# HudsonAlpha/rust-msbwt

Measured on AMD Instinct MI355X. Metric: k-mer count queries/sec (whole node), higher is better.
Workload: dtype u64

## Files before the change

rust-msbwt_amd/csrc/lanes_kernel.hpp:

```cpp
#pragma once
#include <hip/hip_runtime.h>

#include <algorithm>
#include <cstdio>
#include <cstdlib>
#include <type_traits>

#include "kernels.hpp"
#include "rank_ops.hpp"
#include "search_common.hpp"
#include "sparse_table.hpp"

namespace msbwt {
namespace {

typedef __attribute__((address_space(3))) void lds_void;
typedef __attribute__((address_space(1))) const void global_void;

constexpr int kRing = 64;
#ifdef MSBWT_LANES_REGIONS
template <int kWords> constexpr int kRegionsFor = MSBWT_LANES_REGIONS;
#else
template <int kWords> constexpr int kRegionsFor = 10;
#endif
// ... 22 lines not shown

template <int kWords, bool kPlaced, bool kTier = false>
struct LaneScratchT {
    static constexpr int kMaxK = kWords * 32 / 3;
    static constexpr int kRegions = kRegionsFor<kWords>;
    static constexpr int kLineSlots = kRegions * 8;
    static constexpr uint32_t kMaxSecond = uint32_t(kLineSlots) - 64u;
    static_assert(kRegions >= 10 && kRegions % 2 == 0, "first-bound lines take 8 regions; regions come in padded pairs");
    uint4 lines[(kRegions / 2) * 136];
    RingItemT<kWords, kPlaced, kTier> ring[kRing];
    uint32_t cnt[kSearchCounters];
};
static_assert(sizeof(LaneScratchT<6, true>) <= 160 * 1024 / 12 && sizeof(LaneScratchT<6, false, true>) <= 160 * 1024 / 12 && sizeof(LaneScratchT<3, true, true>) <= 160 * 1024 / 12,
              "12 one-wave workgroups per CU (but for packed queries of k > 32 on a two-tier table: 8)");

__host__ __device__ constexpr uint32_t region_base(uint32_t i) { return 136u * (i >> 1) + 72u * (i & 1u); }

__device__ __forceinline__ uint32_t line_base(uint32_t s) { return region_base(s >> 3) + 8u * (s & 7u); }

__device__ __forceinline__ uint32_t xor_and(uint32_t a, uint32_t b, uint32_t c) { return __builtin_amdgcn_bitop3_b32(a, b, c, 0x28); }

struct PlaneLine {
    uint32_t m[8];
    uint32_t meta[8];
};

__device__ __forceinline__ void read_plane_line(const uint4 *lines, uint32_t slot, uint32_t s, PlaneLine &L) {
    const uint32_t base = line_base(slot), g = slot & 7u;
    const uint32_t x0 = (s & 1u) ? 0u : ~0u, x1 = (s & 2u) ? 0u : ~0u, x2 = (s & 4u) ? 0u : ~0u;
#pragma unroll
    for (uint32_t j = 0; j < 8; ++j) {
        const uint4 c = lines[base + (j ^ g)];
        L.m[j] = xor_and(c.z, x2, xor_and(c.y, x1, c.x ^ x0));
        L.meta[j] = c.w;
    }
}

__device__ __forceinline__ uint64_t plane_line_bound(const PlaneLine &L, uint32_t s, uint64_t pos) {
    const uint32_t r = uint32_t(pos) & 255u, idx = r >> 6;
    const uint64_t t = (1ull << (r & 63u)) - 1ull;
    uint32_t cnt = 0, lo = 0;
#pragma unroll
    for (uint32_t j = 0; j < 4; ++j) {
        const uint64_t mask = j < idx ? ~0ull : (j == idx ? t : 0ull);
        cnt += uint32_t(__popc(L.m[2 * j] & uint32_t(mask))) + uint32_t(__popc(L.m[2 * j + 1] & uint32_t(mask >> 32)));
    }
#pragma unroll
    for (uint32_t j = 0; j < 6; ++j) lo = (s == j) ? L.meta[j] : lo;
    const uint32_t hi = (((s >> 2) ? L.meta[7] : L.meta[6]) >> ((s & 3u) * 8u)) & 0xFFu;
    return ((uint64_t(hi) << 32) | lo) + cnt;
}

struct RunCont {
    uint32_t dword, at, acc;
};

__device__ __forceinline__ void run_dword(uint32_t x, uint32_t sx, uint32_t &all, uint32_t &mine) {
    const uint32_t lens = (x >> 3) & 0x1F1F1F1Fu, t = (x & 0x07070707u) ^ sx;
    const uint32_t other = ((t + 0x7F7F7F7Fu) | t) & 0x80808080u;
    const uint32_t match = ((other ^ 0x80808080u) >> 7) * 0xFFu;
    all = __builtin_amdgcn_sad_u8(lens, 0u, 0u);
    mine = __builtin_amdgcn_sad_u8(lens & match, 0u, 0u);
}

__device__ __forceinline__ uint32_t run_dword_clip(uint32_t x, uint32_t s, uint32_t at, uint32_t r) {
    uint32_t cnt = 0;
#pragma unroll
    for (int b = 0; b < 4; ++b) {
        const uint32_t run = (x >> (8 * b)) & 0xFFu, len = run >> 3;
        cnt += (run & 7u) == s ? uint32_t(min(max(int(r) - int(at), 0), int(len))) : 0u;
        at += len;
    }
    return cnt;
}

__device__ __forceinline__ void run_line_first(const uint4 *lines, uint32_t slot, uint32_t s, uint64_t pos, uint64_t &out, uint32_t &need, RunCont &cont) {
    const uint32_t base = line_base(slot), g = slot & 7u;
    const uint4 c0 = lines[base + (0u ^ g)], c1 = lines[base + (1u ^ g)];
    cont = RunCont{24u, 0u, 0u};
    if ((c1.w & 0x80000000u) != 0u) {
        need = lines[base + (2u ^ g)].x * 2u + 1u + ((uint32_t(pos) & 511u) >> 8);
        return;
    }
    const uint32_t lo = s == 0u ? c0.x : s == 1u ? c0.y : s == 2u ? c0.z : s == 3u ? c0.w : s == 4u ? c1.x : c1.y;
    const uint32_t hi = (((s >> 2) ? c1.w : c1.z) >> ((s & 3u) * 8u)) & 0xFFu;
    const uint32_t r0 = uint32_t(pos) & 511u, sx = s * 0x01010101u;
    uint32_t cnt = 0, cur = 0, str = 0;
#pragma unroll
    for (uint32_t j = 2; j < 8; ++j) {
        const uint4 c = lines[base + (j ^ g)];
        const uint32_t word[4] = {c.x, c.y, c.z, c.w};
#pragma unroll
        for (uint32_t i = 0; i < 4; ++i) {
            uint32_t all, mine;
            run_dword(word[i], sx, all, mine);
            const uint32_t end = cur + all;
            cnt += end <= r0 ? mine : 0u;
            const bool here = end > r0 && cont.dword == 24u;
            str = here ? word[i] : str;
            cont.at = here ? cur : cont.at;
            cont.dword = here ? 4u * (j - 2u) + i : cont.dword;
            cur = end;
        }
    }
    cont.acc = cnt;
    out = ((uint64_t(hi) << 32) | lo) + cnt + run_dword_clip(str, s, cont.at, r0);
}

__device__ __forceinline__ void run_line_continue(const uint4 *lines, uint32_t slot, uint32_t s, uint64_t pos, bool same_line, const RunCont &cont, uint64_t &out,
                                                  uint32_t &need) {
    const uint32_t base = line_base(slot), g = slot & 7u;
    const uint4 c0 = lines[base + (0u ^ g)], c1 = lines[base + (1u ^ g)];
    if ((c1.w & 0x80000000u) != 0u) {
        need = lines[base + (2u ^ g)].x * 2u + 1u + ((uint32_t(pos) & 511u) >> 8);
        return;
    }
    const uint32_t lo = s == 0u ? c0.x : s == 1u ? c0.y : s == 2u ? c0.z : s == 3u ? c0.w : s == 4u ? c1.x : c1.y;
    const uint32_t hi = (((s >> 2) ? c1.w : c1.z) >> ((s & 3u) * 8u)) & 0xFFu;
    const uint32_t r1 = uint32_t(pos) & 511u, sx = s * 0x01010101u;
    uint32_t d = same_line ? cont.dword : 0u, cur = same_line ? cont.at : 0u, acc = same_line ? cont.acc : 0u;
    const uint32_t *words = reinterpret_cast<const uint32_t *>(lines);
    while (d < 24u) {
        const uint32_t x = words[(base + ((2u + (d >> 2)) ^ g)) * 4u + (d & 3u)];
        uint32_t all, mine;
        run_dword(x, sx, all, mine);
        if (cur + all <= r1) {
            acc += mine;
            cur += all;
            ++d;
        } else {
            acc += run_dword_clip(x, s, cur, r1);
            break;
        }
    }
    out = ((uint64_t(hi) << 32) | lo) + acc;
}

struct PairLine {
    uint32_t m[4];
    uint32_t field;
};

__device__ __forceinline__ void read_pair_line(const uint4 *lines, uint32_t slot, uint32_t a2, uint32_t b2, PairLine &L) {
    const uint32_t base = line_base(slot), g = slot & 7u, p = a2 * 4u + b2;
    const uint4 a0 = lines[base + (0u ^ g)], a1 = lines[base + (1u ^ g)], b0 = lines[base + (2u ^ g)], b1 = lines[base + (3u ^ g)];
    const uint4 v = lines[base + (uint32_t(kPairValidChunk) ^ g)];
    const uint32_t na0 = (a2 & 1u) - 1u, na1 = ((a2 >> 1) & 1u) - 1u, nb0 = (b2 & 1u) - 1u, nb1 = ((b2 >> 1) & 1u) - 1u;
    L.m[0] = xor_and(b1.x, nb1, xor_and(b0.x, nb0, xor_and(a1.x, na1, xor_and(a0.x, na0, v.x))));
    L.m[1] = xor_and(b1.y, nb1, xor_and(b0.y, nb0, xor_and(a1.y, na1, xor_and(a0.y, na0, v.y))));
    L.m[2] = xor_and(b1.z, nb1, xor_and(b0.z, nb0, xor_and(a1.z, na1, xor_and(a0.z, na0, v.z))));
    L.m[3] = xor_and(b1.w, nb1, xor_and(b0.w, nb0, xor_and(a1.w, na1, xor_and(a0.w, na0, v.w))));
    const uint16_t *halves = reinterpret_cast<const uint16_t *>(lines + base + ((uint32_t(kPairLoChunk) + (p >> 3)) ^ g));
    const uint8_t *bytes = reinterpret_cast<const uint8_t *>(lines + base + (uint32_t(kPairHiChunk) ^ g));
    L.field = uint32_t(halves[p & 7u]) | (uint32_t(bytes[p]) << 16);
}

__device__ __forceinline__ uint32_t pair_line_count(const PairLine &L, uint32_t r) {
    const uint64_t t = (1ull << (r & 63u)) - 1ull;
    const bool upper = r >= 64u;
    const uint64_t lo = upper ? ~0ull : t, hi = upper ? t : 0ull;
    return uint32_t(__popc(L.m[0] & uint32_t(lo))) + uint32_t(__popc(L.m[1] & uint32_t(lo >> 32))) +
           uint32_t(__popc(L.m[2] & uint32_t(hi))) + uint32_t(__popc(L.m[3] & uint32_t(hi >> 32)));
}

__device__ __forceinline__ uint64_t pair_line_bound(const PairLine &L, uint64_t super_base, uint32_t r) {
    return super_base + L.field + pair_line_count(L, r);
}

enum SparseKernel : int { kDirectTable = 0, kSparseComplete = 1, kSparseTier = 2, kSparseWide = 3, kSparseXwide = 4 };

template <int kSparse>
__device__ __forceinline__ constexpr SparseLayout kernel_layout(uint32_t depth) {
    if constexpr (kSparse == kSparseTier) return sparse_layout(depth, true);
    else return kSparse == kSparseXwide ? kLayoutXwide : kSparse == kSparseWide ? kLayoutWide : kLayoutComplete;
}
static_assert(kLayoutTierWide.slots <= kLayoutTier.slots, "kernel_layout<kSparseTier>(kSparseMinDepth) has the most slots of its two");

template <uint32_t kMaxSlots>
__device__ __forceinline__ bool sparse_scan(const uint4 *lines, uint32_t slot, const SparseLayout &L, uint64_t want, uint64_t &l, uint32_t &width, uint32_t &header,
                                            bool &maybe) {
    const uint32_t base = line_base(slot), g = slot & 7u;
    const uint32_t *words = reinterpret_cast<const uint32_t *>(lines);
    const uint8_t *bytes = reinterpret_cast<const uint8_t *>(lines);
    auto word_at = [&](uint32_t w) -> uint32_t { return words[(base + ((w >> 2) ^ g)) * 4u + (w & 3u)]; };
    auto byte_at = [&](uint32_t b) -> uint32_t { return bytes[(base + ((b >> 4) ^ g)) * 16u + (b & 15u)]; };
    auto width_at = [&](uint32_t i) -> uint32_t { return L.width_byte ? byte_at(L.width_byte + i) : word_at(i) >> kSparseWidthShift; };
    auto take = [&](uint32_t i) {
        const uint32_t lo = word_at(L.l_lo_word + i), hi = byte_at(L.l_hi_byte + i);
// ... 130 lines not shown
    auto count_here = [&](int which, uint64_t ballot) {
        if (lane == uint32_t(__builtin_ctzll(__ballot(true)))) ws.cnt[which] += uint32_t(__popcll(ballot));
    };
    const uint32_t dma_group = lane >> 3, dma_chunk_bytes = ((lane & 7u) ^ dma_group) * 16u;

    const uint32_t ncounters = min(uint32_t(kTicketCounters), max(1u, gridDim.x >> 3));
    const uint32_t my_counter = (blockIdx.x >> 3) % ncounters;
    uint64_t static_next = (uint64_t(blockIdx.x) + gridDim.x) * grain;
    auto take_ticket = [&]() -> uint64_t {
        if (tile_counter == nullptr) {
            const uint64_t t = static_next;
            static_next += uint64_t(gridDim.x) * grain;
            return t;
        }
        unsigned long long t = 0;
        if (lane == 0) t = atomicAdd(tile_counter + my_counter * 16u, 1ull);
        const uint64_t drawn = (uint64_t(uint32_t(__builtin_amdgcn_readfirstlane(int(uint32_t(t >> 32))))) << 32) |
                               uint32_t(__builtin_amdgcn_readfirstlane(int(uint32_t(t))));
        return (uint64_t(gridDim.x) + my_counter + drawn * uint64_t(ncounters)) * grain;
    };
    uint64_t next_tile = uint64_t(blockIdx.x) * grain;
    uint32_t seg_left = grain;
    uint64_t seg_after = take_ticket();
    auto advance_tile = [&]() {
        ++next_tile;
        if (--seg_left == 0u) {
            next_tile = seg_after;
            seg_left = grain;
            seg_after = take_ticket();
        }
    };
    uint32_t ring_head = 0, ring_count = 0;
    uint64_t ring_tile = 0;
    uint32_t filter_pause = 0;

    bool have = false;
    bool tmode = false;
    uint32_t tdist = 0;
    bool tmaybe = false;
    bool dmode = false;
    uint32_t ovf_l = 0, ovf_h = 0;
    uint64_t l = 0, h = 0;
    uint32_t w[kWords], rem = 0;
    uint64_t qid = 0;
#pragma unroll
    for (int i = 0; i < kWords; ++i) w[i] = 0;

    uint4 staged_next[kPieces];
#pragma unroll
    for (int i = 0; i < kPieces; ++i) staged_next[i] = make_uint4(0, 0, 0, 0);
    const uint32_t wshift = (kReads && src.strands == 3u) ? 1u : 0u;
    const uint32_t tile_windows = uint32_t(kTile) >> wshift;
    const bool reads_fast = kReads && src.win_off == nullptr && src.windows >= tile_windows;
    const double inv_windows = kReads ? 1.0 / double(src.windows) : 0.0;
    uint32_t staged_n0 = 0;
    uint32_t staged_out = 0, prep_out = 0;
    const bool placed = kPacked && (src.out_index != nullptr || src.place_inline != 0u);
    auto place_of = [&](uint64_t v, uint32_t out) -> uint64_t { return placed ? uint64_t(out) : v; };
    auto fetch_tile_bytes = [&](uint64_t tile, auto first) {
        if (!kPacked && tile >= ntiles) return;
        if (!kReads) {
            if (decltype(first)::value && !kPacked && src.inline_n != 0u) {
                staged_next[0] = lane == 0u ? src.inline_kmer[0] : lane == 1u ? src.inline_kmer[1] : lane == 2u ? src.inline_kmer[2] : lane == 3u ? src.inline_kmer[3] : make_uint4(0, 0, 0, 0);
                return;
            }
            const uint64_t q0 = tile * kTile;
            if constexpr (kPacked) {
                constexpr uint32_t kOwn = kWords == 3 ? 1u : 2u;
                const uint32_t stride = src.packed_stride ? src.packed_stride : kOwn;
                const uint64_t qi = min(q0 + lane, n - 1u);
                const uint64_t *words = reinterpret_cast<const uint64_t *>(kmers) + qi * stride;
                const uint2 a = *reinterpret_cast<const uint2 *>(words);
                staged_next[0].x = a.x;
                staged_next[0].y = a.y;
                if constexpr (kWords == 6) {
                    const uint2 b = *reinterpret_cast<const uint2 *>(words + 1);
                    staged_next[0].z = b.x;
                    staged_next[0].w = b.y;
                }
                const uint32_t *place = src.place_inline != 0u ? reinterpret_cast<const uint32_t *>(words + kOwn)
                                        : src.out_index != nullptr ? src.out_index + qi : reinterpret_cast<const uint32_t *>(words);
                staged_out = *place;
                return;
            }
            const uint32_t nbytes = uint32_t(min(uint64_t(kTile), n - q0)) * k;
#pragma unroll
            for (int i = 0; i < kPieces; ++i) staged_next[i] = load_piece(kmers + q0 * k, nbytes, lane + 64u * i);
        } else if (reads_fast) {
            const uint64_t g0 = (tile * kTile) >> wshift;
            uint64_t r0 = uint64_t(double(g0) * inv_windows);
            int64_t w0 = int64_t(g0 - r0 * src.windows);
            if (w0 < 0) { --r0; w0 += src.windows; }
            if (w0 >= int64_t(src.windows)) { ++r0; w0 -= src.windows; }
            staged_n0 = min(tile_windows, src.windows - uint32_t(w0));
            const uint64_t at = r0 * src.read_len + uint64_t(w0) + 4u * lane, data_len = src.n_reads * src.read_len;
            uint32_t d = 0;
            if (at + 4u <= data_len) {
                __builtin_memcpy(&d, kmers + at, 4);
            } else {
                for (uint32_t b = 0; b < 4u; ++b)
                    if (at + b < data_len) d |= uint32_t(kmers[at + b]) << (8u * b);
            }
            staged_next[0].x = d;
        }
    };
    fetch_tile_bytes(next_tile, std::true_type{});
// ... 111 lines not shown
                        tmode = !dmode;
                    }
                }
                qid = ring_tile * kTile + (it.meta >> 24);
                if constexpr (kPacked) qid = place_of(qid, it.extra[RingItem::kOutAt]);
                ovf_l = ovf_h = 0u;
                have = true;
            }
            const uint32_t taken = min(ring_count, uint32_t(__popcll(idle)));
            ring_head = (ring_head + taken) & (kRing - 1);
            ring_count -= taken;
        }
        const bool broken = have && !(kSparse && tmode) && !(kTier && dmode) && (h > total || l > h);
        if (broken) {
            atomicOr(flags, kFlagInternal);
            if (debug != nullptr && atomicCAS(reinterpret_cast<unsigned long long *>(debug), 0ull, 1ull) == 0ull) {
                debug[1] = l;
                debug[2] = h;
                debug[3] = (uint64_t(rem) << 56) | qid;
                debug[4] = (uint64_t(w[1]) << 32) | w[0];
                debug[5] = (uint64_t(blockIdx.x) << 32) | lane;
            }
            if constexpr (kRange) store_range_raw(src, qid, ~0ull, ~0ull);
            else store_count<kReads>(src, qid, ~0ull);
            have = false;
        }
        busy = __ballot(have);

        if (!prepared && next_tile < ntiles) {
            if (counting && lane == 0u) ws.cnt[kCntWavesWorked] = 1u;
            const uint64_t tile = next_tile;
            advance_tile();
            const uint64_t q0 = tile * kTile;
            const uint32_t in_tile = uint32_t(min(uint64_t(kTile), n - q0));
            const bool filter_now = filter != nullptr && filter_pause == 0;
            bool looked_up = false, passed = false, filtered = false;
            const uint32_t tile_n0 = staged_n0;
            const uint4 packed_words = staged_next[0];
            if constexpr (kPacked) asm volatile("v_mov_b32 %0, %1" : "=v"(prep_out) : "v"(staged_out));
            if (kPacked) {
            } else if (!kReads) {
#pragma unroll
                for (int i = 0; i < kPieces; ++i) ws.lines[kStageLead / 16 + lane + 64u * i] = staged_next[i];
            } else if (reads_fast) {
                const uint32_t d = staged_next[0].x;
                uint32_t f = 0, c = 0;
#pragma unroll
                for (uint32_t b = 0; b < 4u; ++b) {
                    uint32_t sym = (d >> (8u * b)) & 0xFFu;
                    if (src.ascii) sym = ascii_to_code(sym);
                    f |= sym << (8u * b);
                    c |= complement_code(sym) << (8u * (3u - b));
                }
                uint32_t *codes = reinterpret_cast<uint32_t *>(ws.lines) + kStageLead / 4;
                codes[lane] = f;
                codes[64u + (63u - lane)] = c;
            }
            wave_lds_sync();
            prep_kind = 0;
            prep_tile = tile;
            if (lane < in_tile) {
                PackedQuery<kWords> pq;
                if (kPacked) {
                    pack_two_bit<kWords>(k, depth, (uint64_t(packed_words.y) << 32) | packed_words.x, (uint64_t(packed_words.w) << 32) | packed_words.z, pq);
                } else if (!kReads) {
                    pack_query<false, kWords, kReach>(src, depth, stage_bytes + lane * k, q0 + lane, pq);
                } else if (reads_fast) {
                    const uint32_t j = lane >> wshift, o = j + (j >= tile_n0 ? k - 1u : 0u);
                    const bool rc = src.strands == 3u ? (lane & 1u) != 0u : src.strands == 2u;
                    pack_query<false, kWords, kReach>(src, depth, stage_bytes + (rc ? 512u - o - k : o), q0 + lane, pq);
                } else {
                    pack_query<true, kWords, kReach>(src, depth, stage_bytes, q0 + lane, pq);
                }
                if (pq.bad) {
                    if constexpr (kRange) store_range_raw(src, q0 + lane, ~0ull, ~0ull);
                    else store_count<kReads>(src, place_of(q0 + lane, prep_out), ~0ull);
                    atomicOr(flags, kFlagInvalidSymbol);
                } else if (use_table && pq.acgt) {
                    bool maybe = true;
                    if (filter_now) {
                        const uint32_t fi = uint32_t(pq.tidx) & filter_mask;
                        maybe = ((filter[fi >> 5] >> (fi & 31u)) & 1u) != 0u;
                        looked_up = true;
                        passed = maybe;
                    }
                    if (maybe) {
                        if constexpr (kSparse) {
                            const uint64_t x = sparse_mix(pq.tidx, 2u * depth);
                            prep_entry.x = sparse_bucket(x, 2u * depth, sparse_nbuckets);
                            prep_entry.y = sparse_tag(x, layout);
                            prep_entry.z = sparse_tag_hi(x, layout) << 8;
                            if constexpr (kTier) {
                                const uint64_t dk = pq.tidx & dkey_mask, dline = dpacked ? dk / kPackedPerLine : dk >> 3;
                                prep_entry.w = uint32_t(dline);
                                prep_entry.z |= uint32_t(dk - dline * (dpacked ? uint64_t(kPackedPerLine) : 8ull)) << 10;
                            }
                            prep_kind = 3;
                        } else {
                            prep_entry = table_fetch(env, pq.tidx);
                            prep_kind = 1;
                        }
                        prep_q = pq;
                    } else {
                        if constexpr (kRange) store_range_raw(src, q0 + lane, 0ull, 0ull);
                        else store_count<kReads>(src, place_of(q0 + lane, prep_out), 0ull);
                        filtered = true;
                    }
                } else {
                    prep_kind = 2;
                    prep_q = pq;
                }
            }
            if (filter != nullptr) {
                if (filter_now) {
                    const uint32_t nlook = uint32_t(__popcll(__ballot(looked_up))), npass = uint32_t(__popcll(__ballot(passed)));
                    if (nlook > 0 && npass * 10u >= nlook * 9u) filter_pause = 7;
                } else {
                    --filter_pause;
                }
            }
            if (counting) count(kCntTableDecided, __ballot(filtered));
            prepared = true;
            wave_lds_sync();
// ... 181 lines not shown
                    count_here(kCntFirstLines, __ballot(hit && width == kSparseEscapeWidth));
                    count_here(kCntTableDisplaced, __ballot(!hit && have && !fell));
                    count_here(kCntTableDecided, __ballot(!hit && !have));
                    if (kTier) count_here(kCntTierFallbacks, __ballot(fell));
                }
            } else if (kTier && dlooking) {
                const uint32_t base_d = line_base(slot_l), g_d = slot_l & 7u, dslot = uint32_t(h);
                const uint32_t *lw = reinterpret_cast<const uint32_t *>(ws.lines);
                bool esc = false;
                nl = nh = 0;
                step_done = false;
                if (dpacked) {
                    const uint4 c0 = ws.lines[base_d + (0u ^ g_d)];
                    const uint64_t b = (uint64_t(c0.y) << 32) | c0.x;
                    const uint32_t word = 2u + dslot, e = lw[(base_d + ((word >> 2) ^ g_d)) * 4u + (word & 3u)];
                    esc = (b & kPackedEscape) != 0ull;
                    l = esc ? (b & ~kPackedEscape) * kSidePerLine + dslot : b + (e & 0xFFFFu);
                    h = l + (e >> 16);
                } else {
                    const uint4 e = ws.lines[base_d + (dslot ^ g_d)];
                    l = (uint64_t(e.y) << 32) | e.x;
                    h = (uint64_t(e.w) << 32) | e.z;
                }
                if (esc) {
                    uint4 e = dside[l];
                    asm volatile("" : "+v"(e.x), "+v"(e.y), "+v"(e.z), "+v"(e.w));
                    l = (uint64_t(e.y) << 32) | e.x;
                    h = (uint64_t(e.w) << 32) | e.z;
                }
                dmode = false;
                if (l == h) {
                    if constexpr (kRange) store_range_raw(src, qid, 0ull, 0ull);
                    else store_count<kReads>(src, qid, 0ull);
                    have = false;
                }
                if (counting) {
                    count_here(kCntEscapeQueries, __ballot(esc));
                    count_here(kCntFirstLines, __ballot(esc));
                    count_here(kCntTableDecided, __ballot(!have));
                }
            } else if (pair) {
                PairLine L;
                read_pair_line(ws.lines, slot_l, a2, b2, L);
                nl = pair_line_bound(L, super_l, r_l);
                if (second) read_pair_line(ws.lines, slot_h, a2, b2, L);
                asm volatile("" : "+v"(far));
                nh = pair_line_bound(L, far != 0u ? super_far : super_l, r_h);
                consume_symbols<kWords>(w, 6);
                rem -= 2u;
            } else if (!kPair && !kPacked && runs) {
                uint32_t need_l = 0, need_h = 0;
                PlaneLine L;
                nl = nh = 0;
                RunCont cont{24u, 0u, 0u};
                if (ovf_l != 0u) {
                    read_plane_line(ws.lines, slot_l, s1, L);
                    nl = plane_line_bound(L, s1, l);
                } else {
                    run_line_first(ws.lines, slot_l, s1, l, nl, need_l, cont);
                }
                if (ovf_h != 0u) {
                    read_plane_line(ws.lines, slot_h, s1, L);
                    nh = plane_line_bound(L, s1, h);
                } else {
                    run_line_continue(ws.lines, slot_h, s1, h, one_line && ovf_l == 0u, cont, nh, need_h);
                }
                if ((need_l | need_h) != 0u) {
                    ovf_l = ovf_l != 0u ? ovf_l : need_l;
                    ovf_h = ovf_h != 0u ? ovf_h : need_h;
                    step_done = false;
                } else {
                    ovf_l = ovf_h = 0u;
                    consume_symbols<kWords>(w, 3);
                    --rem;
                }
            } else {
                PlaneLine L;
                read_plane_line(ws.lines, slot_l, s1, L);
                nl = plane_line_bound(L, s1, l);
                if (second) read_plane_line(ws.lines, slot_h, s1, L);
                nh = plane_line_bound(L, s1, h);
                consume_symbols<kWords>(w, 3);
                --rem;
            }
            if (step_done) {
                l = nl;
                h = nh;
                if (rem == 0u || l == h) {
                    if constexpr (kRange) store_range(src, qid, l, h);
                    else store_count<kReads>(src, qid, h - l);
                    have = false;
                }
            }
        }
        wave_lds_sync();
    }
    if (counting) {
        wave_lds_sync();
        if (lane < uint32_t(kSearchCounters) && lane != uint32_t(kCntFirstLines))
            atomicAdd(reinterpret_cast<unsigned long long *>(counters + lane), uint64_t(ws.cnt[lane]));
        if (lane == uint32_t(kCntFirstLines)) atomicAdd(reinterpret_cast<unsigned long long *>(counters + lane), uint64_t(ws.cnt[kCntLaneSteps]) + ws.cnt[kCntFirstLines]);
    }
    if (done != nullptr) {
        __threadfence_system();
        if (lane == 0u) __hip_atomic_store(done, done_seq, __ATOMIC_RELEASE, __HIP_MEMORY_SCOPE_SYSTEM);
    }
}

constexpr uint64_t kMaxTiles = 1ull << 32;

template <bool kReads, bool kPair, int kWords, bool kStride96, bool kPacked, int kSparse, bool kRange>
uint32_t resident_waves() {
// ... 74 lines not shown
```

rust-msbwt_amd/csrc/search_common.hpp:

```cpp
#pragma once
#include <hip/hip_runtime.h>

#include <cstdint>

#include "kernels.hpp"
#include "rank_ops.hpp"

namespace msbwt {

struct QuerySource {
    const uint8_t *data;
    uint64_t n;
    uint32_t k;
    uint32_t read_len;
    uint32_t windows;
    uint32_t strands;
    uint32_t ascii;
    uint64_t *out_fwd, *out_rc;
    const uint64_t *read_off, *win_off;
    uint64_t n_reads;
    uint32_t inline_n;
    uint4 inline_kmer[4];
    uint32_t packed;
    const uint32_t *out_index;
// ... 71 lines not shown
    return s == 1u ? 5u : s == 5u ? 1u : s == 2u ? 3u : s == 3u ? 2u : s;
}

template <int kWords>
__device__ __forceinline__ void consume_symbols(uint32_t (&w)[kWords], int bits) {
#pragma unroll
    for (int i = 0; i + 1 < kWords; ++i) w[i] = __builtin_amdgcn_alignbit(w[i + 1], w[i], bits);
    w[kWords - 1] >>= bits;
}

__device__ __forceinline__ uint4 load_piece(const uint8_t *__restrict__ src_bytes, uint32_t nbytes, uint32_t piece) {
    if (piece * 16u >= nbytes) return make_uint4(0, 0, 0, 0);
    if (piece * 16u + 16u <= nbytes) return *reinterpret_cast<const uint4 *>(src_bytes + piece * 16u);
    uint32_t w0 = 0, w1 = 0, w2 = 0, w3 = 0;
    for (uint32_t b = piece * 16u; b < nbytes; ++b) {
        const uint32_t v = uint32_t(src_bytes[b]) << ((b & 3u) * 8u), word = (b & 15u) >> 2;
        if (word == 0u) w0 |= v; else if (word == 1u) w1 |= v; else if (word == 2u) w2 |= v; else w3 |= v;
    }
    return make_uint4(w0, w1, w2, w3);
}

template <bool kReads>
__device__ __forceinline__ void store_count(const QuerySource &src, uint64_t v, uint64_t value) {
    if (!kReads) {
        src.out_fwd[v] = value;
    } else if (src.strands == 3u) {
        ((v & 1u) ? src.out_rc : src.out_fwd)[v >> 1] = value;
    } else {
        (src.strands == 2u ? src.out_rc : src.out_fwd)[v] = value;
    }
}

__device__ __forceinline__ void store_range_raw(const QuerySource &src, uint64_t v, uint64_t l, uint64_t h) {
    const uint64_t at = v * src.range_stride;
    src.out_fwd[at] = l;
    src.out_rc[at] = h;
}
__device__ __forceinline__ void store_range(const QuerySource &src, uint64_t v, uint64_t l, uint64_t h) {
    const bool empty = l == h;
    store_range_raw(src, v, empty ? 0ull : l, empty ? 0ull : h);
}

template <int kBits>
__device__ __forceinline__ void constexpr_shift_or(uint64_t (&bits)[kBits], uint32_t value, uint32_t pos) {
    const uint32_t word = pos >> 6, off = pos & 63u;
#pragma unroll
    for (int j = 0; j < kBits; ++j) {
        if (word == uint32_t(j)) bits[j] |= uint64_t(value) << off;
        if (j > 0 && word == uint32_t(j - 1) && off > 61u) bits[j] |= uint64_t(value) >> (64u - off);
    }
}

template <int kBits>
__device__ __forceinline__ void constexpr_shift_or12(uint64_t (&bits)[kBits], uint32_t value, uint32_t pos) {
    const uint32_t word = pos >> 6, off = pos & 63u;
#pragma unroll
    for (int j = 0; j < kBits; ++j) {
        if (word == uint32_t(j)) bits[j] |= uint64_t(value) << off;
        if (j > 0 && word == uint32_t(j - 1) && off > 52u) bits[j] |= uint64_t(value) >> (64u - off);
    }
}

template <int kWords>
struct PackedQuery {
    static constexpr int kBits = (kWords + 1) / 2;
    uint64_t bits[kBits];
    uint64_t tidx;
    bool bad;
    bool acgt;
};

constexpr uint32_t kStageLead = 64;

__device__ __forceinline__ uint32_t tail_byte_mask(uint32_t d, uint32_t first) {
    const int lo = int(first) - int(4u * d);
    return lo <= 0 ? ~0u : (lo >= 4 ? 0u : (~0u << (8 * lo)));
}

template <int kWords, int kReach = 32>
__device__ __forceinline__ void pack_row_swar(uint32_t k, uint32_t depth, const uint8_t *row, PackedQuery<kWords> &pq) {
    constexpr int kBits = PackedQuery<kWords>::kBits;
    constexpr uint32_t kBlock = kWords == 3 ? 32u : 64u, D = kBlock / 4u;
    uint32_t raw[D];
    __builtin_memcpy(raw, row + k - kBlock, kBlock);
    const uint32_t first_k = kBlock - k, first_d = kBlock - min(depth, k);
#pragma unroll
    for (int j = 0; j < kBits; ++j) pq.bits[j] = 0;
    uint32_t bad = 0, nonacgt = 0;
    uint64_t tidx = 0;
#pragma unroll
    for (uint32_t u = 0; u < D; ++u) {
        const uint32_t d = D - 1u - u;
        const uint32_t x = raw[d] & tail_byte_mask(d, first_k);
        bad |= ((x + 0x7A7A7A7Au) | x) & 0x80808080u;
        const uint32_t y = x & 0x07070707u;
        const uint32_t z = ((y >> 8) | (y << 3)) & 0x003F003Fu;
        const uint32_t g = ((z >> 16) | (z << 6)) & 0xFFFu;
        constexpr_shift_or12<kBits>(pq.bits, g, 12u * u);
        if (u < uint32_t(kReach) / 4u) {
            const uint32_t dm = tail_byte_mask(d, first_d);
            const uint32_t ys = (y & dm) | (0x01010101u & ~dm);
            const uint32_t low2 = ys & 0x03030303u;
            nonacgt |= (low2 - 0x01010101u) & ~low2 & 0x80808080u;
            const uint32_t c = ys - 0x01010101u - ((ys >> 2) & 0x01010101u);
            const uint32_t z2 = ((c >> 8) | (c << 2)) & 0x000F000Fu;
            tidx |= uint64_t(((z2 >> 16) | (z2 << 4)) & 0xFFu) << (8u * u);
        }
    }
    pq.tidx = tidx & ((1ull << (2u * min(depth, uint32_t(kReach >= 32 ? 31 : kReach)))) - 1ull);
    pq.bad = bad != 0u;
    pq.acgt = nonacgt == 0u;
}

template <int kWords>
__device__ __forceinline__ void pack_two_bit(uint32_t k, uint32_t depth, uint64_t lo, uint64_t hi, PackedQuery<kWords> &pq) {
    constexpr int kBits = PackedQuery<kWords>::kBits;
    constexpr uint32_t kMaxK = kWords == 3 ? 32u : 64u;
#pragma unroll
    for (int j = 0; j < kBits; ++j) pq.bits[j] = 0;
    if (k < 32u) lo &= (1ull << (2u * k)) - 1ull;
    if (k < 64u && k > 32u) hi &= (1ull << (2u * (k - 32u))) - 1ull;
    if (k <= 32u) hi = 0ull;
#pragma unroll
    for (uint32_t u = 0; u < kMaxK / 4u; ++u) {
        const uint32_t x = uint32_t((u < 8u ? lo : hi) >> (8u * (u & 7u))) & 0xFFu;
        const uint32_t y = (x & 0x03u) | ((x & 0x0Cu) << 1) | ((x & 0x30u) << 2) | ((x & 0xC0u) << 3);
        const uint32_t g = y + 0x249u + ((y & (y >> 1)) & 0x249u);
        constexpr_shift_or12<kBits>(pq.bits, g, 12u * u);
    }
    const uint32_t reach = min(depth, k);
    pq.tidx = reach >= 32u ? lo : (lo & ((1ull << (2u * reach)) - 1ull));
    pq.bad = false;
    pq.acgt = true;
}

template <bool kReads, int kWords, int kReach = 32>
__device__ __forceinline__ void pack_query(const QuerySource &src, uint32_t depth, const uint8_t *staged, uint64_t v,
                                           PackedQuery<kWords> &pq) {
    if constexpr (!kReads) {
        (void)v;
        pack_row_swar<kWords, kReach>(src.k, depth, staged, pq);
        return;
    }
    constexpr int kBits = PackedQuery<kWords>::kBits;
    constexpr uint32_t kBlock = kWords == 3 ? 32u : 64u;
    const uint32_t k = src.k;
    uint32_t raw[kBlock / 4];
    bool rc = false;
    if (!kReads) {
        __builtin_memcpy(raw, staged + k - kBlock, kBlock);
    } else {
        const uint64_t g = src.strands == 3u ? (v >> 1) : v;
        rc = src.strands == 3u ? (v & 1u) != 0 : src.strands == 2u;
        uint64_t first, data_len;
        if (src.win_off == nullptr) {
            first = (g / src.windows) * src.read_len + (g % src.windows);
            data_len = src.n_reads * src.read_len;
        } else {
            uint64_t lo = 0, hi = src.n_reads;
            while (hi - lo > 1) {
                const uint64_t mid = (lo + hi) >> 1;
                if (src.win_off[mid] <= g) lo = mid; else hi = mid;
            }
            first = src.read_off[lo] + (g - src.win_off[lo]);
// ... 123 lines not shown
```

Measured before the change: 33.52 billion.

## Rework run-length line rank with scaled-length dot products and wave-uniform continue

Rewrites the run-length encoded line rank. Run lengths are kept scaled by 8 so per-dword sums and symbol-matched counts come from sad_u8 and udot4, and the partial-dword clip becomes branchless byte arithmetic. The continue path now resumes from the cached dword and loops under a wave ballot instead of a per-lane while loop, while a cold line uses a compact full scan. The first-line scan unroll depends on kWords. This cuts ALU work and divergence per rank but adds registers for the extra cached word, and the counts must stay exact after the >>6 rescaling.

```diff
diff --git a/rust-msbwt_amd/csrc/lanes_kernel.hpp b/rust-msbwt_amd/csrc/lanes_kernel.hpp
--- a/rust-msbwt_amd/csrc/lanes_kernel.hpp
+++ b/rust-msbwt_amd/csrc/lanes_kernel.hpp
@@ -98,88 +98,103 @@
 }
 
 struct RunCont {
-    uint32_t dword, at, acc;
+    uint32_t dword, at8, acc64, x;
 };
 
-__device__ __forceinline__ void run_dword(uint32_t x, uint32_t sx, uint32_t &all, uint32_t &mine) {
-    const uint32_t lens = (x >> 3) & 0x1F1F1F1Fu, t = (x & 0x07070707u) ^ sx;
-    const uint32_t other = ((t + 0x7F7F7F7Fu) | t) & 0x80808080u;
-    const uint32_t match = ((other ^ 0x80808080u) >> 7) * 0xFFu;
-    all = __builtin_amdgcn_sad_u8(lens, 0u, 0u);
-    mine = __builtin_amdgcn_sad_u8(lens & match, 0u, 0u);
-}
-
-__device__ __forceinline__ uint32_t run_dword_clip(uint32_t x, uint32_t s, uint32_t at, uint32_t r) {
-    uint32_t cnt = 0;
-#pragma unroll
-    for (int b = 0; b < 4; ++b) {
-        const uint32_t run = (x >> (8 * b)) & 0xFFu, len = run >> 3;
-        cnt += (run & 7u) == s ? uint32_t(min(max(int(r) - int(at), 0), int(len))) : 0u;
-        at += len;
-    }
-    return cnt;
-}
-
+__device__ __forceinline__ uint32_t run_match8(uint32_t x, uint32_t sx) {
+    const uint32_t t = (x & 0x07070707u) ^ sx;
+    return ~(t + 0x07070707u) & 0x08080808u;
+}
+
+__device__ __forceinline__ bool run_dword_take(uint32_t x, uint32_t sx, uint32_t r8, bool live, uint32_t cur8, uint32_t &end8, uint32_t &acc64) {
+    const uint32_t len8 = x & 0xF8F8F8F8u;
+    end8 = __builtin_amdgcn_sad_u8(len8, 0u, cur8);
+    const bool whole = end8 <= r8 && live;
+    acc64 = __builtin_amdgcn_udot4(len8, whole ? run_match8(x, sx) : 0u, acc64, false);
+    return whole;
+}
+
+__device__ __forceinline__ uint32_t run_dword_clip(uint32_t x, uint32_t sx, uint32_t t) {
+    const uint32_t lens = (x >> 3) & 0x1F1F1F1Fu, two = lens + (lens << 8), incl = two + (two << 16);
+    const uint32_t tb = __builtin_amdgcn_perm(t, t, 0u);
+    const uint32_t ge = ((incl | 0x80808080u) - tb) & 0x80808080u, low7 = ge - (ge >> 7);
+    const uint32_t q = (tb & low7) | (incl & ~low7);
+    return __builtin_amdgcn_udot4(q - (q << 8), run_match8(x, sx), 0u, false);
+}
+
+__device__ __forceinline__ uint32_t run_home(uint32_t s) { return line_base(s) + (s & 7u); }
+
+__device__ __forceinline__ uint32_t run_word(const uint4 *lines, uint32_t home, uint32_t d) {
+    const uint32_t *words = reinterpret_cast<const uint32_t *>(lines);
+    const uint32_t x = words[(home * 4u) ^ (min(d, 23u) + 8u)];
+    return d < 24u ? x : 0u;
+}
+
+template <int kPerTurn>
+__device__ __forceinline__ void run_line_scan(const uint4 *lines, uint32_t home, uint32_t sx, uint32_t r8, uint32_t &whole, uint32_t &at8, uint32_t &cnt64) {
+    uint32_t cur = 0;
+    whole = at8 = cnt64 = 0;
+#pragma unroll kPerTurn
+    for (uint32_t j = 2; j < 8; ++j) {
+        const uint4 c = lines[home ^ j];
+        const uint32_t word[4] = {c.x, c.y, c.z, c.w};
+#pragma unroll
+        for (uint32_t i = 0; i < 4; ++i) {
+            uint32_t end;
+            const bool took = run_dword_take(word[i], sx, r8, true, cur, end, cnt64);
+            whole += took ? 1u : 0u;
+            at8 = took ? end : at8;
+            cur = end;
+        }
+    }
+}
+
+template <int kPerTurn>
 __device__ __forceinline__ void run_line_first(const uint4 *lines, uint32_t slot, uint32_t s, uint64_t pos, uint64_t &out, uint32_t &need, RunCont &cont) {
-    const uint32_t base = line_base(slot), g = slot & 7u;
-    const uint4 c0 = lines[base + (0u ^ g)], c1 = lines[base + (1u ^ g)];
-    cont = RunCont{24u, 0u, 0u};
+    const uint32_t home = run_home(slot);
+    const uint4 c0 = lines[home], c1 = lines[home ^ 1u];
+    cont = RunCont{24u, 0u, 0u, 0u};
     if ((c1.w & 0x80000000u) != 0u) {
-        need = lines[base + (2u ^ g)].x * 2u + 1u + ((uint32_t(pos) & 511u) >> 8);
+        need = lines[home ^ 2u].x * 2u + 1u + ((uint32_t(pos) & 511u) >> 8);
         return;
     }
     const uint32_t lo = s == 0u ? c0.x : s == 1u ? c0.y : s == 2u ? c0.z : s == 3u ? c0.w : s == 4u ? c1.x : c1.y;
     const uint32_t hi = (((s >> 2) ? c1.w : c1.z) >> ((s & 3u) * 8u)) & 0xFFu;
-    const uint32_t r0 = uint32_t(pos) & 511u, sx = s * 0x01010101u;
-    uint32_t cnt = 0, cur = 0, str = 0;
-#pragma unroll
-    for (uint32_t j = 2; j < 8; ++j) {
-        const uint4 c = lines[base + (j ^ g)];
-        const uint32_t word[4] = {c.x, c.y, c.z, c.w};
-#pragma unroll
-        for (uint32_t i = 0; i < 4; ++i) {
-            uint32_t all, mine;
-            run_dword(word[i], sx, all, mine);
-            const uint32_t end = cur + all;
-            cnt += end <= r0 ? mine : 0u;
-            const bool here = end > r0 && cont.dword == 24u;
-            str = here ? word[i] : str;
-            cont.at = here ? cur : cont.at;
-            cont.dword = here ? 4u * (j - 2u) + i : cont.dword;
-            cur = end;
-        }
-    }
-    cont.acc = cnt;
-    out = ((uint64_t(hi) << 32) | lo) + cnt + run_dword_clip(str, s, cont.at, r0);
+    const uint32_t r8 = (uint32_t(pos) & 511u) * 8u, sx = s * 0x01010101u;
+    uint32_t cnt, at, whole;
+    run_line_scan<kPerTurn>(lines, home, sx, r8, whole, at, cnt);
+    const uint32_t x = run_word(lines, home, whole);
+    cont = RunCont{whole, at, cnt, x};
+    out = ((uint64_t(hi) << 32) | lo) + ((cnt + 8u * run_dword_clip(x, sx, min((r8 - at) >> 3, 127u))) >> 6);
 }
 
 __device__ __forceinline__ void run_line_continue(const uint4 *lines, uint32_t slot, uint32_t s, uint64_t pos, bool same_line, const RunCont &cont, uint64_t &out,
                                                   uint32_t &need) {
-    const uint32_t base = line_base(slot), g = slot & 7u;
-    const uint4 c0 = lines[base + (0u ^ g)], c1 = lines[base + (1u ^ g)];
+    const uint32_t home = run_home(slot);
+    const uint4 c0 = lines[home], c1 = lines[home ^ 1u];
     if ((c1.w & 0x80000000u) != 0u) {
-        need = lines[base + (2u ^ g)].x * 2u + 1u + ((uint32_t(pos) & 511u) >> 8);
+        need = lines[home ^ 2u].x * 2u + 1u + ((uint32_t(pos) & 511u) >> 8);
         return;
     }
     const uint32_t lo = s == 0u ? c0.x : s == 1u ? c0.y : s == 2u ? c0.z : s == 3u ? c0.w : s == 4u ? c1.x : c1.y;
     const uint32_t hi = (((s >> 2) ? c1.w : c1.z) >> ((s & 3u) * 8u)) & 0xFFu;
-    const uint32_t r1 = uint32_t(pos) & 511u, sx = s * 0x01010101u;
-    uint32_t d = same_line ? cont.dword : 0u, cur = same_line ? cont.at : 0u, acc = same_line ? cont.acc : 0u;
-    const uint32_t *words = reinterpret_cast<const uint32_t *>(lines);
-    while (d < 24u) {
-        const uint32_t x = words[(base + ((2u + (d >> 2)) ^ g)) * 4u + (d & 3u)];
-        uint32_t all, mine;
-        run_dword(x, sx, all, mine);
-        if (cur + all <= r1) {
-            acc += mine;
-            cur += all;
-            ++d;
-        } else {
-            acc += run_dword_clip(x, s, cur, r1);
-            break;
-        }
-    }
-    out = ((uint64_t(hi) << 32) | lo) + acc;
+    const uint32_t r8 = (uint32_t(pos) & 511u) * 8u, sx = s * 0x01010101u;
+    uint32_t d, cur, acc, x;
+    if (same_line) {
+        d = cont.dword, cur = cont.at8, acc = cont.acc64, x = cont.x;
+        bool more;
+        do {
+            uint32_t end;
+            more = run_dword_take(x, sx, r8, d < 24u, cur, end, acc);
+            cur = more ? end : cur;
+            d += more ? 1u : 0u;
+            x = run_word(lines, home, d);
+        } while (__ballot(more) != 0ull);
+    } else {
+        run_line_scan<1>(lines, home, sx, r8, d, cur, acc);
+        x = run_word(lines, home, d);
+    }
+    out = ((uint64_t(hi) << 32) | lo) + ((acc + 8u * run_dword_clip(x, sx, min((r8 - cur) >> 3, 127u))) >> 6);
 }
 
 struct PairLine {
@@ -937,12 +952,12 @@
                 uint32_t need_l = 0, need_h = 0;
                 PlaneLine L;
                 nl = nh = 0;
-                RunCont cont{24u, 0u, 0u};
+                RunCont cont{24u, 0u, 0u, 0u};
                 if (ovf_l != 0u) {
                     read_plane_line(ws.lines, slot_l, s1, L);
                     nl = plane_line_bound(L, s1, l);
                 } else {
-                    run_line_first(ws.lines, slot_l, s1, l, nl, need_l, cont);
+                    run_line_first<kWords == 3 ? 6 : 3>(ws.lines, slot_l, s1, l, nl, need_l, cont);
                 }
                 if (ovf_h != 0u) {
                     read_plane_line(ws.lines, slot_h, s1, L);
```

Measured after the change: 32.43 billion. 3.2% lower.

## Stage read windows as pre-packed 3-bit/2-bit span streams in LDS

Applied to the files above, without the earlier changes.

In the fast reads path, each lane now writes its 4 forward and 4 complement symbols into LDS as pre-packed bit streams: 3-bit codes, 2-bit table indices and validity flags. It does this with atomicOr into a span area that is cleared first. Each query window is then extracted with funnel shifts (alignbit) instead of re-packing k bytes per lane. When only the table index is needed, the 3-bit code extraction is skipped. The cost is an extra clear plus a barrier and LDS atomics during staging.

```diff
diff --git a/rust-msbwt_amd/csrc/lanes_kernel.hpp b/rust-msbwt_amd/csrc/lanes_kernel.hpp
--- a/rust-msbwt_amd/csrc/lanes_kernel.hpp
+++ b/rust-msbwt_amd/csrc/lanes_kernel.hpp
@@ -416,6 +416,9 @@
     const uint32_t wshift = (kReads && src.strands == 3u) ? 1u : 0u;
     const uint32_t tile_windows = uint32_t(kTile) >> wshift;
     const bool reads_fast = kReads && src.win_off == nullptr && src.windows >= tile_windows;
+    [[maybe_unused]] uint32_t *span_area = reinterpret_cast<uint32_t *>(ws.lines) + kStageLead / 4;
+    static_assert(kStageLead % 8u == 0u && kStageLead + 4u * kSpanDwords <= 640u, "the span's streams: 8-byte reads, inside the part of the line area that staging has always used");
+    [[maybe_unused]] const bool index_only = kReads && kWords == 3 && kSparse != kDirectTable && !kTier && use_table && k == depth && kSideFetch && table_side != nullptr;
     const double inv_windows = kReads ? 1.0 / double(src.windows) : 0.0;
     uint32_t staged_n0 = 0;
     uint32_t staged_out = 0, prep_out = 0;
@@ -633,9 +636,12 @@
                     f |= sym << (8u * b);
                     c |= complement_code(sym) << (8u * (3u - b));
                 }
-                uint32_t *codes = reinterpret_cast<uint32_t *>(ws.lines) + kStageLead / 4;
-                codes[lane] = f;
-                codes[64u + (63u - lane)] = c;
+                static_assert(kSpanZeroed == uint32_t(kTile), "one cleared dword per lane");
+                uint32_t lane_here = lane;
+                if constexpr (kWords == 6) asm volatile("" : "+v"(lane_here));
+                span_area[lane_here] = 0u;
+                wave_lds_sync();
+                stage_span_lane(span_area, lane_here, f, c);
             }
             wave_lds_sync();
             prep_kind = 0;
@@ -649,7 +655,9 @@
                 } else if (reads_fast) {
                     const uint32_t j = lane >> wshift, o = j + (j >= tile_n0 ? k - 1u : 0u);
                     const bool rc = src.strands == 3u ? (lane & 1u) != 0u : src.strands == 2u;
-                    pack_query<false, kWords, kReach>(src, depth, stage_bytes + (rc ? 512u - o - k : o), q0 + lane, pq);
+                    uint32_t k_here = k, depth_here = depth;
+                    if constexpr (kWords == 6) asm volatile("" : "+s"(k_here), "+s"(depth_here));
+                    pack_span_window<kWords, kReach>(k_here, depth_here, span_area, rc ? o : 512u - o - k, index_only, pq);
                 } else {
                     pack_query<true, kWords, kReach>(src, depth, stage_bytes, q0 + lane, pq);
                 }
diff --git a/rust-msbwt_amd/csrc/search_common.hpp b/rust-msbwt_amd/csrc/search_common.hpp
--- a/rust-msbwt_amd/csrc/search_common.hpp
+++ b/rust-msbwt_amd/csrc/search_common.hpp
@@ -147,7 +147,7 @@
 }
 
 template <int kBits>
-__device__ __forceinline__ void constexpr_shift_or12(uint64_t (&bits)[kBits], uint32_t value, uint32_t pos) {
+__host__ __device__ __forceinline__ void constexpr_shift_or12(uint64_t (&bits)[kBits], uint32_t value, uint32_t pos) {
     const uint32_t word = pos >> 6, off = pos & 63u;
 #pragma unroll
     for (int j = 0; j < kBits; ++j) {
@@ -167,13 +167,13 @@
 
 constexpr uint32_t kStageLead = 64;
 
-__device__ __forceinline__ uint32_t tail_byte_mask(uint32_t d, uint32_t first) {
+__host__ __device__ __forceinline__ uint32_t tail_byte_mask(uint32_t d, uint32_t first) {
     const int lo = int(first) - int(4u * d);
     return lo <= 0 ? ~0u : (lo >= 4 ? 0u : (~0u << (8 * lo)));
 }
 
 template <int kWords, int kReach = 32>
-__device__ __forceinline__ void pack_row_swar(uint32_t k, uint32_t depth, const uint8_t *row, PackedQuery<kWords> &pq) {
+__host__ __device__ __forceinline__ void pack_row_swar(uint32_t k, uint32_t depth, const uint8_t *row, PackedQuery<kWords> &pq) {
     constexpr int kBits = PackedQuery<kWords>::kBits;
     constexpr uint32_t kBlock = kWords == 3 ? 32u : 64u, D = kBlock / 4u;
     uint32_t raw[D];
@@ -205,6 +205,98 @@
     pq.tidx = tidx & ((1ull << (2u * min(depth, uint32_t(kReach >= 32 ? 31 : kReach)))) - 1ull);
     pq.bad = bad != 0u;
     pq.acgt = nonacgt == 0u;
+}
+
+constexpr uint32_t kSpanCodes3 = 0;
+constexpr uint32_t kSpanPairs = 56;
+constexpr uint32_t kSpanDwords = kSpanPairs + 2 * 40;
+constexpr uint32_t kSpanZeroed = 64;
+static_assert(kSpanZeroed >= kSpanPairs, "codes3 is ORed into a cleared stream");
+
+__host__ __device__ __forceinline__ uint32_t low_mask_dword(uint32_t nbits, uint32_t j) {
+    const int n = int(nbits) - int(32u * j);
+    return n <= 0 ? 0u : (n >= 32 ? ~0u : ((1u << n) - 1u));
+}
+
+__host__ __device__ __forceinline__ uint32_t funnel_right(uint32_t hi, uint32_t lo, uint32_t sh) {
+#if defined(__HIP_DEVICE_COMPILE__)
+    return __builtin_amdgcn_alignbit(hi, lo, sh);
+#else
+    return uint32_t(((uint64_t(hi) << 32) | lo) >> (sh & 31u));
+#endif
+}
+
+__host__ __device__ __forceinline__ void span_groups(uint32_t x, uint32_t &g3, uint32_t &g2, uint32_t &gf) {
+    const uint32_t y = x & 0x07070707u;
+    const uint32_t z = ((y >> 8) | (y << 3)) & 0x003F003Fu;
+    g3 = ((z >> 16) | (z << 6)) & 0xFFFu;
+    const uint32_t c = (y + 0x03030303u - ((y >> 2) & 0x01010101u)) & 0x03030303u;
+    const uint32_t z2 = ((c >> 8) | (c << 2)) & 0x000F000Fu;
+    g2 = ((z2 >> 16) | (z2 << 4)) & 0xFFu;
+    const uint32_t big = (((x & 0x7F7F7F7Fu) + 0x7A7A7A7Au) | x) & 0x80808080u;
+    const uint32_t none = ~((x & 0x03030303u) + 0x03030303u) & 0x04040404u;
+    const uint32_t f = (big >> 7) | (none >> 1);
+    const uint32_t zf = ((f >> 8) | (f << 2)) & 0x000F000Fu;
+    gf = ((zf >> 16) | (zf << 4)) & 0xFFu;
+}
+
+__host__ __device__ __forceinline__ void stage_span_lane(uint32_t *area, uint32_t lane, uint32_t fwd, uint32_t comp) {
+    uint8_t *bytes = reinterpret_cast<uint8_t *>(area + kSpanPairs);
+#pragma unroll
+    for (uint32_t half = 0; half < 2u; ++half) {
+        const uint32_t group = half == 0u ? lane : 127u - lane;
+        uint32_t g3, g2, gf;
+        span_groups(half == 0u ? comp : fwd, g3, g2, gf);
+        const uint32_t bit = 12u * group, word = bit >> 5;
+        const uint64_t v = uint64_t(g3) << (bit & 31u);
+#if defined(__HIP_DEVICE_COMPILE__)
+        atomicOr(area + kSpanCodes3 + word, uint32_t(v));
+        atomicOr(area + kSpanCodes3 + word + 1u, uint32_t(v >> 32));
+#else
+        area[kSpanCodes3 + word] |= uint32_t(v);
+        area[kSpanCodes3 + word + 1u] |= uint32_t(v >> 32);
+#endif
+        bytes[8u * (group >> 2) + (group & 3u)] = uint8_t(g2);
+        bytes[8u * (group >> 2) + 4u + (group & 3u)] = uint8_t(gf);
+    }
+}
+
+template <int kWords, int kReach = 32>
+__host__ __device__ __forceinline__ void pack_span_window(uint32_t k, uint32_t depth, const uint32_t *area, uint32_t q, bool index_only, PackedQuery<kWords> &pq) {
+    constexpr int kBits = PackedQuery<kWords>::kBits;
+    constexpr uint32_t kFlagDwords = kWords == 3 ? 2u : 4u;
+    const uint32_t reach = min(min(depth, k), uint32_t(kReach >= 32 ? 31 : kReach));
+    const uint32_t at2 = (2u * q) >> 5, sh2 = (2u * q) & 31u;
+    const uint2 *pairs = reinterpret_cast<const uint2 *>(area + kSpanPairs) + at2;
+    uint32_t c2[3], fl[kFlagDwords + 1u];
+#pragma unroll
+    for (uint32_t j = 0; j <= kFlagDwords; ++j) {
+        const uint2 p = pairs[j];
+        if (j < 3u) c2[j] = p.x;
+        fl[j] = p.y;
+    }
+    const uint32_t t0 = funnel_right(c2[1], c2[0], sh2) & low_mask_dword(2u * reach, 0u), t1 = funnel_right(c2[2], c2[1], sh2) & low_mask_dword(2u * reach, 1u);
+    pq.tidx = (uint64_t(t1) << 32) | t0;
+    uint32_t bad = 0, nonacgt = 0;
+#pragma unroll
+    for (uint32_t j = 0; j < kFlagDwords; ++j) {
+        const uint32_t v = funnel_right(fl[j + 1u], fl[j], sh2);
+        bad |= v & 0x55555555u & low_mask_dword(2u * k, j);
+        if (j < 2u) nonacgt |= v & 0xAAAAAAAAu & low_mask_dword(2u * reach, j);
+    }
+    pq.bad = bad != 0u;
+    pq.acgt = nonacgt == 0u;
+#pragma unroll
+    for (int j = 0; j < kBits; ++j) pq.bits[j] = 0;
+    if (!index_only || !pq.acgt) {
+        const uint32_t at3 = (3u * q) >> 5, sh3 = (3u * q) & 31u;
+        const uint32_t *codes3 = area + kSpanCodes3 + at3;
+        uint32_t d[kWords + 1];
+#pragma unroll
+        for (int j = 0; j <= kWords; ++j) d[j] = codes3[j];
+#pragma unroll
+        for (int j = 0; j < kWords; ++j) pq.bits[j >> 1] |= uint64_t(funnel_right(d[j + 1], d[j], sh3) & low_mask_dword(3u * k, uint32_t(j))) << (32 * (j & 1));
+    }
 }
 
 template <int kWords>
```

New measurement: 34.62 billion before, 32.17 billion after. -7.1%, worse.
